# simonsobs/Pixell.jl

Measured on AMD Instinct MI355X. Metric: Mpix/s CAR bilinear reproject (Float64) + % HBM roofline, 1/2/4/8 MI355X, higher is better.
Workload: dtype f64

## Files before the change

### include/pixell_hip.h

```cpp
#ifndef PIXELL_HIP_H
#define PIXELL_HIP_H

#include <stddef.h>
#include <stdint.h>

#ifdef __cplusplus
extern "C" {
#endif

#define PXL_VERSION 100

typedef struct pxl_car_wcs {
    double cdelt[2];
    double crpix[2];
    double crval[2];
    double unit;
} pxl_car_wcs;

#define PXL_OK         0
#define PXL_EINVAL   (-22)
#define PXL_ENOMEM   (-12)
#define PXL_EHIP     (-5)
#define PXL_ENODEV   (-19)

// ... 39 lines not shown
int pxl_pix2sky_tan_f64(const pxl_car_wcs* wcs, int64_t n, const double* ipix, const double* jpix,
                        double* ra, double* dec, void* stream);
int pxl_posmap_tan_f64(const pxl_car_wcs* wcs, const int64_t shape[2], int64_t row0, int64_t nrows,
                       double* ra, double* dec, void* stream);

typedef struct pxl_reproject_plan pxl_reproject_plan;

int pxl_reproject_plan_create(const pxl_car_wcs* wcs_in, const int64_t shape_in[3],
                              int64_t src_row0, int64_t src_nrows,
                              const pxl_car_wcs* wcs_out, const int64_t shape_out[2],
                              int64_t dst_row0, int64_t dst_nrows,
                              pxl_reproject_plan** plan);
int pxl_reproject_execute(pxl_reproject_plan* plan, const double* src, double* dst, void* stream);
int pxl_reproject_build_tables(pxl_reproject_plan* plan, void* stream);
int pxl_reproject_execute_rows(pxl_reproject_plan* plan, const double* src, double* dst,
                               int64_t r0, int64_t nr, void* stream);
int pxl_reproject_execute_f32(pxl_reproject_plan* plan, const float* src, float* dst, void* stream);
int pxl_reproject_execute_rows_f32(pxl_reproject_plan* plan, const float* src, float* dst,
                                   int64_t r0, int64_t nr, void* stream);
int pxl_reproject_plan_src_rows(const pxl_reproject_plan* plan, int64_t* lo, int64_t* hi);
int pxl_reproject_plan_rows_covered(const pxl_reproject_plan* plan, int64_t have_lo, int64_t have_hi,
                                    int64_t* lo, int64_t* hi);
int pxl_reproject_plan_set_variant(pxl_reproject_plan* plan, int variant);
int pxl_reproject_plan_destroy(pxl_reproject_plan* plan);

typedef struct pxl_halo_xfer {
    int32_t peer;
    int32_t reserved;
    int64_t row0;
    int64_t nrows;
} pxl_halo_xfer;
int pxl_reproject_sharded_step_f64(pxl_reproject_plan* plan, double* src, double* dst,
                                   int64_t own_row0, int64_t own_nrows,
                                   const pxl_halo_xfer* sends, int nsends, const pxl_halo_xfer* recvs, int nrecvs,
                                   void* rccl_comm, void* stream);
int pxl_reproject_sharded_step_f32(pxl_reproject_plan* plan, float* src, float* dst,
                                   int64_t own_row0, int64_t own_nrows,
                                   const pxl_halo_xfer* sends, int nsends, const pxl_halo_xfer* recvs, int nrecvs,
                                   void* rccl_comm, void* stream);

#define PXL_COMM_ID_BYTES 128
int pxl_comm_unique_id(void* id128);
int pxl_comm_init_rank(const void* id128, int rank, int nranks, void** comm);
int pxl_comm_destroy(void* comm);
const char* pxl_comm_backend(void);

// ... 112 lines not shown
```

### pixell.jl_amd/_lib.py

```python
import ctypes as C
import os

_HERE = os.path.dirname(os.path.abspath(__file__))
LIB_PATH = os.environ.get("PXL_LIB_PATH", os.path.join(_HERE, "libpixell_hip.so"))

WRAP_NONE, WRAP_REWIND, WRAP_UNWIND = 0, 1, 2
FORM_RECIP, FORM_DIV, FORM_RECIP_AV = 0, 1, 2


class PixellHipError(RuntimeError):

    def __init__(self, code, message):
        super().__init__("libpixell_hip error %d: %s" % (code, message))
        self.code = code


class CarWCSStruct(C.Structure):
    _fields_ = [("cdelt", C.c_double * 2), ("crpix", C.c_double * 2), ("crval", C.c_double * 2),
                ("unit", C.c_double)]


_P = C.c_void_p
_I64 = C.c_int64
_WP = C.POINTER(CarWCSStruct)
# ... 5 lines not shown
    "pxl_device_count": (C.c_int, []),
    "pxl_release_scratch": (C.c_int, []),
    "pxl_pix2sky_car_f64": (C.c_int, [_WP, _I64, _P, _P, C.c_int, _P]),
    "pxl_rewind_f64": (C.c_int, [_P, _I64, C.c_double, C.c_double, _P]),
    "pxl_unwind_f64": (C.c_int, [_P, _I64, C.c_int, C.c_double, C.c_double, _P]),
    "pxl_pix2sky_car_soa_f64": (C.c_int, [_WP, _I64, _P, _P, _P, _P, C.c_int, _P]),
    "pxl_sky2pix_car_f64": (C.c_int, [_WP, _SHP, _I64, _P, _P, C.c_int, C.c_int, _P]),
    "pxl_sky2pix_car_soa_f64": (C.c_int, [_WP, _SHP, _I64, _P, _P, _P, _P, C.c_int, C.c_int, _P]),
    "pxl_posmap_car_f64": (C.c_int, [_WP, _SHP, _I64, _I64, _P, _P, C.c_int, _P]),
    "pxl_pixareamap_car_f64": (C.c_int, [_WP, _SHP, _I64, _I64, _P, _P]),
    "pxl_distance_transform_car_f64": (C.c_int, [_WP, _SHP, _P, _P, _P]),
    "pxl_sky2pix_tan_f64": (C.c_int, [_WP, _I64, _P, _P, _P, _P, _P]),
    "pxl_pix2sky_tan_f64": (C.c_int, [_WP, _I64, _P, _P, _P, _P, _P]),
    "pxl_posmap_tan_f64": (C.c_int, [_WP, _SHP, _I64, _I64, _P, _P, _P]),
    "pxl_reproject_plan_create": (C.c_int, [_WP, _SHP, _I64, _I64, _WP, _SHP, _I64, _I64, C.POINTER(_P)]),
    "pxl_reproject_execute": (C.c_int, [_P, _P, _P, _P]),
    "pxl_reproject_build_tables": (C.c_int, [_P, _P]),
    "pxl_reproject_execute_rows": (C.c_int, [_P, _P, _P, _I64, _I64, _P]),
    "pxl_reproject_execute_f32": (C.c_int, [_P, _P, _P, _P]),
    "pxl_reproject_execute_rows_f32": (C.c_int, [_P, _P, _P, _I64, _I64, _P]),
    "pxl_reproject_plan_src_rows": (C.c_int, [_P, C.POINTER(_I64), C.POINTER(_I64)]),
    "pxl_reproject_plan_rows_covered": (C.c_int, [_P, _I64, _I64, C.POINTER(_I64), C.POINTER(_I64)]),
    "pxl_reproject_plan_set_variant": (C.c_int, [_P, C.c_int]),
    "pxl_reproject_plan_destroy": (C.c_int, [_P]),
    "pxl_reproject_sharded_step_f64": (C.c_int, [_P, _P, _P, _I64, _I64, _P, C.c_int, _P, C.c_int, _P, _P]),
    "pxl_reproject_sharded_step_f32": (C.c_int, [_P, _P, _P, _I64, _I64, _P, C.c_int, _P, C.c_int, _P, _P]),
    "pxl_comm_unique_id": (C.c_int, [_P]),
    "pxl_comm_init_rank": (C.c_int, [_P, C.c_int, C.c_int, C.POINTER(_P)]),
    "pxl_comm_destroy": (C.c_int, [_P]),
    "pxl_comm_backend": (C.c_char_p, []),
    "pxl_reproject_car_bilinear_f64": (C.c_int, [_WP, _SHP, _P, _WP, _SHP, _P, _P]),
    "pxl_reproject_generic_bilinear_f64": (C.c_int, [_WP, C.c_int, _SHP, _P, _WP, C.c_int, _SHP, _P, _P]),
    "pxl_reproject_generic_last_tiles": (C.c_int, [C.POINTER(_I64), C.POINTER(_I64), _P]),
    "pxl_generic_plan_create": (C.c_int, [_WP, C.c_int, _SHP, _WP, C.c_int, _SHP, _P, C.POINTER(_P)]),
    "pxl_generic_plan_execute": (C.c_int, [_P, _I64, _P, _P, _P]),
    "pxl_generic_plan_tiles": (C.c_int, [_P, C.POINTER(_I64), C.POINTER(_I64)]),
    "pxl_generic_plan_destroy": (C.c_int, [_P]),
    "pxl_sample_car_bilinear_f64": (C.c_int, [_WP, _SHP, _P, _I64, _I64, _I64, _P, _P, _P]),
    "pxl_sample_car_bilinear_f32": (C.c_int, [_WP, _SHP, _P, _I64, _I64, _I64, _P, _P, _P]),
    "pxl_scatter_car_bilinear_f64": (C.c_int, [_WP, _SHP, _P, _I64, _I64, _I64, _P, _P, _P]),
    "pxl_sample_pairs_elems": (_I64, [_SHP, _I64]),
    "pxl_sample_build_pairs_f64": (C.c_int, [_SHP, _P, _I64, _P, _P]),
    "pxl_sample_build_pairs_f32": (C.c_int, [_SHP, _P, _I64, _P, _P]),
    "pxl_sample_car_bilinear_pairs_f64": (C.c_int, [_WP, _SHP, _P, _I64, _I64, _I64, _P, _P, _P]),
    "pxl_sample_car_bilinear_pairs_f32": (C.c_int, [_WP, _SHP, _P, _I64, _I64, _I64, _P, _P, _P]),
    "pxl_spline_prefilter_car_f64": (C.c_int, [_WP, _SHP, _P, _P, _P]),
# ... 78 lines not shown
```

### pixell.jl_amd/csrc/pxl_kernels.hip

```cpp
#include <hip/hip_runtime.h>

#include <algorithm>
#include <mutex>
#include <vector>
#include <cmath>
#include <cstdarg>
#include <cstdio>
#include <cstring>
#include <new>
#include <type_traits>

#include "pxl_device.h"

using namespace pxl;

static thread_local char g_err[512] = "";

static int fail(int code, const char* fmt, ...) {
    va_list ap;
    va_start(ap, fmt);
    vsnprintf(g_err, sizeof(g_err), fmt, ap);
    va_end(ap);
    return code;
}
#define HIP_TRY(expr)                                                                         \
// ... 32 lines not shown
    const char* v = getenv(name);
    return (v && *v) ? atoi(v) : dflt;
}

#include "pxl_elementwise.h"
#include "pxl_unwrap.h"
#include "pxl_maps.h"
#include "pxl_fastmath.h"
#include "pxl_tan.h"
#include "pxl_reproject.h"
#include "pxl_reproject_dma.h"
#include "pxl_sample.h"
#include "pxl_scatter.h"
#include "pxl_misc.h"
#include "pxl_rccl.h"
#include "pxl_spread.h"
#include "pxl_distance.h"
#include "pxl_spline.h"
#include "pxl_pol.h"
#include "pxl_polsolve.h"

static constexpr size_t PXL_RING_BYTES = 17 * 1024;
static constexpr int64_t PXL_MIN_TILES = 8192;

struct Tables { double* xfx; double* yfy; int32_t* xi0; int32_t* yj0; size_t bytes; };
static Tables table_layout(void* mem, int64_t nxo, int64_t nyo) {
    auto up16 = [](size_t b) { return (b + 15) & ~(size_t)15; };
    const uintptr_t xfx = (uintptr_t)mem, yfy = xfx + up16((size_t)nxo * 8), xi0 = yfy + up16((size_t)nyo * 8),
                    yj0 = xi0 + up16((size_t)nxo * 4);
    return {(double*)xfx, (double*)yfy, (int32_t*)xi0, (int32_t*)yj0, (size_t)(yj0 + up16((size_t)nyo * 4) - xfx)};
}
static void launch_build_tables(const pxl_car_wcs& win, int64_t nx, int64_t ny, const pxl_car_wcs& wout, int64_t nxo, int64_t nyo,
                                const Tables& t, hipStream_t st) {
    hipLaunchKernelGGL(k_build_tables, dim3(stream_grid(nxo + nyo, 256)), dim3(256), 0, st, car_affine(wout),
                       sky2pix_setup(win, nx, ny, 1, PXL_FORM_DIV), nxo, nyo, t.xi0, t.xfx, t.yj0, t.yfy);
}

struct SlotRule { int cw; double slack; int64_t align; };
static constexpr SlotRule kSlot64 = {128, 5.0, 2};
static constexpr SlotRule kSlot32 = {256, 8.0, 4};
static int64_t seg_for(const SlotRule& r, int pairs, double sx) {
    double span = ceil((double)(r.cw * pairs) * sx) + r.slack;
    return ((int64_t)span + (r.align - 1)) & ~(r.align - 1);
}
static bool stageable(const SlotRule& r, int64_t sg, bool periodic, int64_t nx, double sy) {
    return (sg <= PXL_MAXCH * r.cw) && !(periodic && sg > nx) && sy <= 3.0;
// ... 3 lines not shown
    pxl_car_wcs win, wout;
    int64_t nx, ny, nc, src_row0, src_nrows;
    int64_t nxo, nyo, dst_row0, dst_nrows;
    int periodic;
    int device;
    Tables tab;
    void* table_mem;
    int32_t* h_yj0;
    int variant;
    int pairs;
    int pairs_dma;
    int seg_dma;
    int pairs_dma32;
    int seg_dma32;
    bool dma32_ok;
    int dypos;
    int rh;
    int rh32;
    int seg;
    int dxpos;
    int ns, pf;
    int nt;
    double* zero_page;
    bool staged_ok;
    bool vec_load;
    bool tables_built;
    hipStream_t comm_stream;
    hipEvent_t ev_ready, ev_halo;
    int64_t cov_have_lo, cov_have_hi, cov_lo, cov_hi;
};

struct DeviceState {
    hipMemPool_t pool;
    unsigned int* last_exact;
    int64_t generic_tiles;
};
static std::mutex g_dev_mu;
static DeviceState g_dev[64] = {};
static DeviceState* device_state() {
    int dev = 0;
    if (hipGetDevice(&dev) != hipSuccess || dev < 0 || dev >= 64) return nullptr;
    return &g_dev[dev];
}

static hipMemPool_t scratch_pool() {
    DeviceState* d = device_state();
    if (!d) return nullptr;
    std::lock_guard<std::mutex> lock(g_dev_mu);
    if (!d->pool) {
// ... 163 lines not shown
    if (items < (int64_t)min_per_front * fronts) fronts = 1;
    int64_t per = (items + fronts - 1) / fronts;
    if (cap > 0 && per * fronts > cap) { fronts = 1; per = items; }
    return {fronts, per};
}

static int check_rows(const char* who, const int64_t shape[2], int64_t row0, int64_t nrows) {
    if (!shape || shape[0] < 1 || shape[1] < 1) return fail(PXL_EINVAL, "%s: bad shape", who);
    if (row0 < 0 || nrows < 0 || row0 + nrows > shape[1])
        return fail(PXL_EINVAL, "%s: rows [%lld, %lld) outside the map (ny=%lld)", who, (long long)row0,
                    (long long)(row0 + nrows), (long long)shape[1]);
    return PXL_OK;
}

template <class T>
static int reproject_rows_impl(pxl_reproject_plan* pl, const T* src, T* dst, int64_t r0, int64_t nr, void* stream) {
    if (!pl) return fail(PXL_EINVAL, "execute: null plan");
    if (r0 < 0 || nr < 0 || r0 + nr > pl->dst_nrows) return fail(PXL_EINVAL, "execute: rows outside the dst window");
    if (nr == 0) return PXL_OK;
    if (!dst || (!src && pl->src_nrows > 0)) return fail(PXL_EINVAL, "execute: null src/dst");
    if (!pl->tables_built) return fail(PXL_EINVAL, "execute_rows: tables not built");
    hipStream_t st = (hipStream_t)stream;
    constexpr bool f32 = std::is_same<T, float>::value;

    ReprojParams p;
    memset(&p, 0, sizeof(p));
    p.src = src; p.dst = dst;
    p.xi0 = pl->tab.xi0; p.xfx = pl->tab.xfx; p.yj0 = pl->tab.yj0; p.yfy = pl->tab.yfy;
    p.nx = pl->nx; p.ny = pl->ny; p.src_row0 = pl->src_row0; p.src_nrows = pl->src_nrows;
    p.nxo = pl->nxo; p.dst_row0 = pl->dst_row0; p.dst_nrows = pl->dst_nrows;
    p.r0 = r0; p.nr = nr; p.nc = (int32_t)pl->nc; p.periodic = pl->periodic;

    const bool aligned = (((uintptr_t)src & 15) == 0);
    bool staged = f32 ? (pl->dma32_ok && aligned) : pl->staged_ok;
    if (pl->variant == 1) staged = false;
    if (!staged) {
        int64_t work = ((pl->nxo + 1) / 2) * nr;
        dim3 g(stream_grid(work, 256), (unsigned)pl->nc);
        hipLaunchKernelGGL((k_reproject_gather<T>), g, dim3(256), 0, st, p);
        return check_launch("k_reproject_gather");
    }

    const bool vec = f32 ? true : (pl->vec_load && aligned);
    const bool use_dma = f32 ? true : (vec && pl->variant != 2);
    const int pairs = f32 ? pl->pairs_dma32 : (use_dma ? pl->pairs_dma : pl->pairs);
    const int cw = f32 ? kSlot32.cw : kSlot64.cw;
    const int TW = cw * pairs;
    p.seg = f32 ? pl->seg_dma32 : (use_dma ? pl->seg_dma : pl->seg);
    p.dxpos = pl->dxpos; p.dypos = pl->dypos;
    p.ntx = (int32_t)((pl->nxo + TW - 1) / TW);
    int rh = f32 ? pl->rh32 : pl->rh;
    while (rh > 4 && (int64_t)p.ntx * ((nr + rh - 1) / rh) * pl->nc < PXL_MIN_TILES) rh >>= 1;
    p.rh = rh;
    p.nty = (int32_t)((nr + rh - 1) / rh);
    p.ntiles = (int64_t)p.ntx * p.nty * pl->nc;
    p.tiles_per_xcd = (p.ntiles + 7) / 8;
    const int64_t nblocks = 8 * p.tiles_per_xcd;
    if (nblocks > 0x7fffffffLL) return fail(PXL_EINVAL, "execute: too many tiles (%lld)", (long long)nblocks);
    dim3 grid((unsigned)nblocks), block(64);
    if (use_dma) {
        const size_t esz = sizeof(T);
        p.ns = pl->ns; p.pf = pl->pf; p.zero_page = pl->zero_page;
        p.nt = pl->nt != 0;
        while ((size_t)p.ns * p.seg * esz > PXL_RING_BYTES && p.ns > 4) p.ns >>= 1;
        size_t dma_lds = (size_t)p.ns * (size_t)p.seg * esz;
        const int nch = (p.seg + cw - 1) / cw;
        return launch_reproject_dma_t<T>(pairs, nch, grid, dma_lds, st, p);
    }
    size_t lds_bytes = (size_t)PXL_NS * (size_t)pl->seg * sizeof(double);
    if (pl->pairs == 2) {
        if (vec) hipLaunchKernelGGL((k_reproject_staged<2, true>), grid, block, lds_bytes, st, p);
        else     hipLaunchKernelGGL((k_reproject_staged<2, false>), grid, block, lds_bytes, st, p);
    } else {
        if (vec) hipLaunchKernelGGL((k_reproject_staged<1, true>), grid, block, lds_bytes, st, p);
        else     hipLaunchKernelGGL((k_reproject_staged<1, false>), grid, block, lds_bytes, st, p);
    }
    return check_launch("k_reproject_staged");
}

template <class T>
static int sharded_step_impl(pxl_reproject_plan* pl, T* src, T* dst, int64_t own_row0, int64_t own_nrows,
                             const pxl_halo_xfer* sends, int nsends, const pxl_halo_xfer* recvs, int nrecvs,
                             void* comm, void* stream) {
    if (!pl || !src || !dst) return fail(PXL_EINVAL, "sharded_step: null plan or buffer");
    if (nsends < 0 || nrecvs < 0 || (nsends > 0 && !sends) || (nrecvs > 0 && !recvs)) return fail(PXL_EINVAL, "sharded_step: bad transfer lists");
    const int64_t lo = pl->src_row0, hi = pl->src_row0 + pl->src_nrows;
    if (own_row0 < lo || own_nrows < 0 || own_row0 + own_nrows > hi) return fail(PXL_EINVAL, "sharded_step: owned rows outside the plan's source window");
    hipStream_t st = (hipStream_t)stream;
    int rc = PXL_OK;
    const bool exchange = nsends + nrecvs > 0;
// ... 513 lines not shown
    if (shape_in[0] < 1 || shape_in[1] < 1 || shape_in[2] < 1 || shape_out[0] < 1 || shape_out[1] < 1)
        return fail(PXL_EINVAL, "plan_create: shapes must be positive");
    if (shape_in[0] > 400000000 || shape_in[1] > 1000000000 || shape_out[0] > 1000000000 || shape_out[1] > 1000000000)
        return fail(PXL_EINVAL, "plan_create: axis too long (source RA axis <= 4e8, others <= 1e9 pixels)");
    if (src_row0 < 0 || src_nrows < 0 || src_row0 + src_nrows > shape_in[1])
        return fail(PXL_EINVAL, "plan_create: source window outside the map");
    if (dst_row0 < 0 || dst_nrows < 0 || dst_row0 + dst_nrows > shape_out[1])
        return fail(PXL_EINVAL, "plan_create: destination window outside the map");

    pxl_reproject_plan* pl = new (std::nothrow) pxl_reproject_plan();
    if (!pl) return fail(PXL_ENOMEM, "plan_create: host allocation failed");
    pl->cov_lo = 0; pl->cov_hi = -1;
    pl->win = *wcs_in; pl->wout = *wcs_out;
    pl->nx = shape_in[0]; pl->ny = shape_in[1]; pl->nc = shape_in[2];
    pl->src_row0 = src_row0; pl->src_nrows = src_nrows;
    pl->nxo = shape_out[0]; pl->nyo = shape_out[1];
    pl->dst_row0 = dst_row0; pl->dst_nrows = dst_nrows;
    pl->periodic = car_periodic(wcs_in, pl->nx);
    pl->tables_built = false;

    hipError_t e = hipGetDevice(&pl->device);
    if (e != hipSuccess) { delete pl; return fail(PXL_ENODEV, "hipGetDevice: %s", hipGetErrorString(e)); }

    const size_t nyo = (size_t)pl->nyo, off_zero = table_layout(nullptr, pl->nxo, pl->nyo).bytes, total = off_zero + 64;
    e = hipMalloc(&pl->table_mem, total);
    if (e != hipSuccess) { delete pl; return fail(PXL_ENOMEM, "plan_create: hipMalloc(%zu): %s", total, hipGetErrorString(e)); }
    char* base = (char*)pl->table_mem;
    e = hipMemset(base + off_zero, 0, 64);
    if (e != hipSuccess) { (void)hipFree(pl->table_mem); delete pl; return fail(PXL_EHIP, "plan_create: hipMemset: %s", hipGetErrorString(e)); }
    pl->zero_page = (double*)(base + off_zero);
    pl->tab = table_layout(base, pl->nxo, pl->nyo);

    pl->h_yj0 = new (std::nothrow) int32_t[nyo];
    if (!pl->h_yj0) { (void)hipFree(pl->table_mem); delete pl; return fail(PXL_ENOMEM, "plan_create: host allocation failed"); }
    CarAffine co = car_affine(pl->wout);
    Sky2Pix si = sky2pix_setup(pl->win, pl->nx, pl->ny, 1, PXL_FORM_DIV);
    for (int64_t j = 0; j < pl->nyo; ++j) {
        double fr;
        split_cell(s2p_y(si, p2s_dec(co, (double)(j + 1))), &pl->h_yj0[j], &fr);
    }

    double sx = fabs((pl->wout.cdelt[0] * pl->wout.unit) / (pl->win.cdelt[0] * pl->win.unit));
    pl->dxpos = ((pl->wout.cdelt[0] * pl->wout.unit) / (pl->win.cdelt[0] * pl->win.unit)) > 0 ? 1 : 0;
    pl->dypos = ((pl->wout.cdelt[1] * pl->wout.unit) / (pl->win.cdelt[1] * pl->win.unit)) > 0 ? 1 : 0;
    double sy = fabs((pl->wout.cdelt[1] * pl->wout.unit) / (pl->win.cdelt[1] * pl->win.unit));
    pl->rh = env_int("PXL_REPROJECT_RH", sy >= 1.5 ? 4 : (sy > 0.3 ? 16 : 8));
    if (pl->rh < 1) pl->rh = 1;
    if (pl->rh > 64) pl->rh = 64;
    pl->rh32 = env_int("PXL_REPROJECT_RH", 32);
    if (pl->rh32 < 1) pl->rh32 = 1;
    if (pl->rh32 > 64) pl->rh32 = 64;
    pl->ns = env_int("PXL_REPROJECT_NS", (double)pl->nx * (double)pl->ny * (double)pl->nc * 8.0 <= 128.0 * 1048576.0 ? 4 : 8);
    if (pl->ns < 4) pl->ns = 4;
// ... 7 lines not shown
    if (pl->pf < 0) pl->pf = 0;
    const int max_seg = PXL_MAXCH * kSlot64.cw;
    int want = env_int("PXL_REPROJECT_PAIRS", sx <= 0.55 ? 4 : 2);
    if (want != 1 && want != 2 && want != 4) want = 2;
    pl->pairs_dma = want;
    while (pl->pairs_dma > 1 && seg_for(kSlot64, pl->pairs_dma, sx) > max_seg) pl->pairs_dma >>= 1;
    const int64_t seg_dma = seg_for(kSlot64, pl->pairs_dma, sx);
    pl->seg_dma = (int)std::min<int64_t>(seg_dma, max_seg);
    pl->pairs = want > 2 ? 2 : want;
    if (seg_for(kSlot64, pl->pairs, sx) > max_seg && pl->pairs == 2) pl->pairs = 1;
    int64_t seg = seg_for(kSlot64, pl->pairs, sx);
    pl->staged_ok = stageable(kSlot64, seg, pl->periodic, pl->nx, sy) && stageable(kSlot64, seg_dma, pl->periodic, pl->nx, sy);
    pl->seg = (int)(seg <= max_seg ? seg : max_seg);
    {
        const int max_seg32 = PXL_MAXCH * kSlot32.cw;
        pl->pairs_dma32 = env_int("PXL_REPROJECT_PAIRS", sx < 0.75 ? 1 : 2);
        if (pl->pairs_dma32 != 1 && pl->pairs_dma32 != 2 && pl->pairs_dma32 != 4) pl->pairs_dma32 = 2;
        while (pl->pairs_dma32 > 1 && seg_for(kSlot32, pl->pairs_dma32, sx) > max_seg32) pl->pairs_dma32 >>= 1;
        int64_t s32 = seg_for(kSlot32, pl->pairs_dma32, sx);
        pl->dma32_ok = stageable(kSlot32, s32, pl->periodic, pl->nx, sy) && (pl->nx % 4 == 0);
        pl->seg_dma32 = (int)std::min<int64_t>(s32, max_seg32);
    }
    pl->vec_load = (pl->nx % 2 == 0);
    *out = pl;
    return PXL_OK;
}

int pxl_reproject_plan_set_variant(pxl_reproject_plan* pl, int variant) {
    if (!pl || variant < 0 || variant > 2) return fail(PXL_EINVAL, "set_variant: bad argument");
    pl->variant = variant;
    return PXL_OK;
}

int pxl_reproject_plan_destroy(pxl_reproject_plan* pl) {
    if (!pl) return PXL_OK;
    if (pl->comm_stream) {
        (void)hipStreamSynchronize(pl->comm_stream);
        (void)hipEventDestroy(pl->ev_ready);
        (void)hipEventDestroy(pl->ev_halo);
        (void)hipStreamDestroy(pl->comm_stream);
    }
    if (pl->table_mem) (void)hipFree(pl->table_mem);
    delete[] pl->h_yj0;
    delete pl;
    return PXL_OK;
}

int pxl_reproject_build_tables(pxl_reproject_plan* pl, void* stream) {
    if (!pl) return fail(PXL_EINVAL, "build_tables: null plan");
    launch_build_tables(pl->win, pl->nx, pl->ny, pl->wout, pl->nxo, pl->nyo, pl->tab, (hipStream_t)stream);
    int rc = check_launch("k_build_tables");
    if (rc == PXL_OK) pl->tables_built = true;
    return rc;
}

int pxl_reproject_execute_rows(pxl_reproject_plan* pl, const double* src, double* dst, int64_t r0, int64_t nr,
                               void* stream) {
    return reproject_rows_impl(pl, src, dst, r0, nr, stream);
}

int pxl_reproject_execute_rows_f32(pxl_reproject_plan* pl, const float* src, float* dst, int64_t r0, int64_t nr,
                                   void* stream) {
    return reproject_rows_impl(pl, src, dst, r0, nr, stream);
}

int pxl_reproject_execute(pxl_reproject_plan* pl, const double* src, double* dst, void* stream) {
    int rc = pxl_reproject_build_tables(pl, stream);
    if (rc) return rc;
    return pxl_reproject_execute_rows(pl, src, dst, 0, pl->dst_nrows, stream);
}

int pxl_reproject_execute_f32(pxl_reproject_plan* pl, const float* src, float* dst, void* stream) {
    int rc = pxl_reproject_build_tables(pl, stream);
    if (rc) return rc;
    return pxl_reproject_execute_rows_f32(pl, src, dst, 0, pl->dst_nrows, stream);
// ... 494 lines not shown
```

### pixell.jl_amd/csrc/pxl_reproject.h

```cpp
#pragma once

__global__ __launch_bounds__(256) void k_build_tables(CarAffine out, Sky2Pix in, int64_t nxo, int64_t nyo,
                                                      int32_t* __restrict__ xi0, double* __restrict__ xfx,
                                                      int32_t* __restrict__ yj0, double* __restrict__ yfy) {
    int64_t stride = (int64_t)gridDim.x * blockDim.x;
    for (int64_t k = (int64_t)blockIdx.x * blockDim.x + threadIdx.x; k < nxo + nyo; k += stride) {
        if (k < nxo) {
            double a = p2s_ra(out, (double)(k + 1));
            split_cell(s2p_x(in, a), &xi0[k], &xfx[k]);
        } else {
            int64_t j = k - nxo;
            double d = p2s_dec(out, (double)(j + 1));
            split_cell(s2p_y(in, d), &yj0[j], &yfy[j]);
        }
    }
}

struct ReprojParams {
    const void* src;
    void* dst;
    const int32_t* xi0; const double* xfx;
    const int32_t* yj0; const double* yfy;
    int64_t nx, ny, src_row0, src_nrows;
    int64_t nxo, dst_row0, dst_nrows;
    int64_t r0, nr;
    int32_t nc, periodic;
    int32_t rh;
    int32_t seg;
    int32_t dxpos;
    int32_t dypos;
    int32_t ntx, nty;
    int64_t ntiles, tiles_per_xcd;
    int32_t ns, pf;
    int32_t nt;
    const double* zero_page;
};

__device__ inline int64_t xcd_tile(int64_t b, int64_t tiles_per_xcd) {
    return (b & 7) * tiles_per_xcd + (b >> 3);
}

template <typename T>
__global__ __launch_bounds__(256) void k_reproject_gather(ReprojParams p) {
    const int64_t npair = (p.nxo + 1) / 2;
    const int64_t total = npair * p.nr;
    const int c = blockIdx.y;
    SrcViewT<T> m{(const T*)p.src + (int64_t)c * p.nx * p.src_nrows, p.nx, p.ny, p.src_row0, p.src_nrows, p.periodic};
    T* dplane = (T*)p.dst + (int64_t)c * p.nxo * p.dst_nrows;
    int64_t stride = (int64_t)gridDim.x * blockDim.x;
    for (int64_t t = (int64_t)blockIdx.x * blockDim.x + threadIdx.x; t < total; t += stride) {
        int64_t rr = t / npair;
        int64_t i = (t - rr * npair) * 2;
        int64_t r = p.r0 + rr;
        int64_t j0 = p.yj0[p.dst_row0 + r];
        double fy = p.yfy[p.dst_row0 + r];
        int64_t o = r * p.nxo + i;
        dplane[o] = (T)bilerp_cells(m, p.xi0[i], p.xfx[i], j0, fy);
        if (i + 1 < p.nxo) dplane[o + 1] = (T)bilerp_cells(m, p.xi0[i + 1], p.xfx[i + 1], j0, fy);
// ... 185 lines not shown
```

### pixell.jl_amd/csrc/pxl_reproject_dma.h

```cpp
#pragma once

template <int N>
__device__ __forceinline__ void wait_vm() {
    asm volatile("s_waitcnt vmcnt(%0)" ::"n"(N) : "memory");
}

__device__ __forceinline__ void wait_vm_upto(int k) {
    if (k < 8) {
        if (k < 4) {
            if (k < 2) { if (k < 1) wait_vm<0>(); else wait_vm<1>(); }
            else       { if (k < 3) wait_vm<2>(); else wait_vm<3>(); }
        } else {
            if (k < 6) { if (k < 5) wait_vm<4>(); else wait_vm<5>(); }
            else       { if (k < 7) wait_vm<6>(); else wait_vm<7>(); }
        }
    } else if (k < 16) {
        if (k < 12) {
            if (k < 10) { if (k < 9) wait_vm<8>(); else wait_vm<9>(); }
            else        { if (k < 11) wait_vm<10>(); else wait_vm<11>(); }
        } else {
            if (k < 14) { if (k < 13) wait_vm<12>(); else wait_vm<13>(); }
            else        { if (k < 15) wait_vm<14>(); else wait_vm<15>(); }
        }
    } else {
        if (k < 24) { if (k < 20) wait_vm<16>(); else wait_vm<20>(); }
        else        { if (k < 32) wait_vm<24>(); else wait_vm<32>(); }
    }
}

__device__ __forceinline__ void glds16_saddr(const void* sbase, uint32_t voff, uint32_t lds_byte_addr) {
    asm volatile("s_mov_b32 m0, %2\n\ts_nop 4\n\tglobal_load_lds_dwordx4 %1, %0"
                 :: "s"(sbase), "v"(voff), "s"(lds_byte_addr) : "memory");
}
__device__ __forceinline__ void glds16_vaddr(const void* gsrc, uint32_t lds_byte_addr) {
    asm volatile("s_mov_b32 m0, %1\n\ts_nop 0\n\tglobal_load_lds_dwordx4 %0, off"
                 :: "v"(gsrc), "s"(lds_byte_addr) : "memory");
}

template <typename T, int PAIRS, int NCH>
__global__ __launch_bounds__(64) void k_reproject_dma(ReprojParams p) {
    extern __shared__ __attribute__((aligned(16))) unsigned char lds_raw[];
    T* const lds = reinterpret_cast<T*>(lds_raw);
    const int lane = threadIdx.x;
    constexpr int EPL = 16 / (int)sizeof(T);
    constexpr int CW = 64 * EPL;
    constexpr int TW = CW * PAIRS;

    const int64_t t = xcd_tile(blockIdx.x, p.tiles_per_xcd);
    if (t >= p.ntiles) return;
    const int tx = (int)(t % p.ntx);
    const int64_t trest = t / p.ntx;
    const int ty = (int)(trest % p.nty);
    const int c = (int)(trest / p.nty);

    const T* splane = (const T*)p.src + (int64_t)c * p.nx * p.src_nrows;
    T* dplane = (T*)p.dst + (int64_t)c * p.nxo * p.dst_nrows;

    const int64_t c0 = (int64_t)tx * TW;
    const int64_t clast = (c0 + TW < p.nxo ? c0 + TW : p.nxo) - 1;
    const int64_t rb = p.r0 + (int64_t)ty * p.rh;
    const int64_t re = (rb + p.rh < p.r0 + p.nr) ? rb + p.rh : p.r0 + p.nr;
    const int nrows = (int)(re - rb);

    const int64_t a = p.dxpos ? p.xi0[c0] : p.xi0[clast];
    const int64_t ua = a - 1;
    const int64_t cbase0 = ua - (((ua % EPL) + EPL) % EPL);
    int dloc[PAIRS][EPL];
    double fx[PAIRS][EPL];
    bool act[PAIRS][EPL];
    bool fits = true;
#pragma unroll
    for (int q = 0; q < PAIRS; ++q) {
// ... 17 lines not shown
    const int dir = p.dypos ? 1 : -1;
    const int my_t0 = p.dypos ? my_j0 : -(my_j0 + 1);
    const double my_wa = p.dypos ? 1 - my_fy : my_fy;
    const double my_wb = p.dypos ? my_fy : 1 - my_fy;
    {
        int nxt = __shfl_down(my_t0, 1, 64);
        bool mono = (lane + 1 >= nrows) || (nxt >= my_t0);
        if (!mono) fits = false;
    }

    if (!__all(fits)) {
        SrcViewT<T> m{splane, p.nx, p.ny, p.src_row0, p.src_nrows, p.periodic};
        for (int64_t r = rb; r < re; ++r) {
            int64_t j0 = p.yj0[p.dst_row0 + r];
            double fy = p.yfy[p.dst_row0 + r];
#pragma unroll
            for (int q = 0; q < PAIRS; ++q)
#pragma unroll
                for (int e = 0; e < EPL; ++e) {
                    int64_t col = c0 + q * CW + EPL * lane + e;
                    if (act[q][e]) dplane[r * p.nxo + col] = (T)bilerp_cells(m, p.xi0[col], fx[q][e], j0, fy);
                }
        }
        return;
    }

    uint32_t voff[NCH];
#pragma unroll
    for (int ch = 0; ch < NCH; ++ch) {
        int64_t u = cbase0 + ch * CW + EPL * lane;
        bool ok = true;
        if (p.periodic) { u %= p.nx; if (u < 0) u += p.nx; }
        else ok = (u >= 0) && (u < p.nx);
        voff[ch] = ok ? (uint32_t)(u * (int64_t)sizeof(T)) : 0xFFFFFFFFu;
    }

    const uint32_t lds_base = (uint32_t)(uintptr_t)lds;
    const uint32_t slot_bytes = (uint32_t)p.seg * (uint32_t)sizeof(T);
    const int ns_mask = p.ns - 1;

    int tv_lo = 1, tv_hi = 0;
    {
        const int64_t jlo = (p.src_row0 + 1 > 1) ? p.src_row0 + 1 : 1;
        const int64_t jhi = (p.src_row0 + p.src_nrows < p.ny) ? p.src_row0 + p.src_nrows : p.ny;
        if (jhi >= jlo) {
            if (p.dypos) { tv_lo = (int)jlo; tv_hi = (int)jhi; } else { tv_lo = -(int)jhi; tv_hi = -(int)jlo; }
        }
// ... 35 lines not shown

    const bool vec_store = ((p.nxo % EPL) == 0) && (((uintptr_t)p.dst & 15) == 0);
    T* orow = dplane + rb * p.nxo + c0 + EPL * lane;

    double hA[PAIRS][EPL], hB[PAIRS][EPL], wx[PAIRS][EPL];
#pragma unroll
    for (int q = 0; q < PAIRS; ++q)
#pragma unroll
        for (int e = 0; e < EPL; ++e) { wx[q][e] = 1 - fx[q][e]; hA[q][e] = 0.0; hB[q][e] = 0.0; }
    auto hrow = [&](int tr, double (&h)[PAIRS][EPL]) {
        const T* R = lds + (tr & ns_mask) * p.seg;
#pragma unroll
        for (int q = 0; q < PAIRS; ++q)
#pragma unroll
            for (int e = 0; e < EPL; ++e) {
                const int d = dloc[q][e];
                h[q][e] = wx[q][e] * (double)R[d] + fx[q][e] * (double)R[d + 1];
            }
    };
    auto row_loop = [&](auto fast_tag, auto nt_tag) {
    constexpr bool FAST = decltype(fast_tag)::value;
    constexpr bool NT = decltype(nt_tag)::value;
    int th = INT32_MIN / 2;
    for (int rr = 0; rr < nrows; ++rr) {
        const int t0 = __builtin_amdgcn_readlane(my_t0, rr);
        {
            const int ra = (rr + p.pf < nrows) ? rr + p.pf : nrows - 1;
            int tmax = __builtin_amdgcn_readlane(my_t0, ra) + 1;
            const int tlim = t0 + p.ns - 1;
            if (tmax > tlim) tmax = tlim;
            while (treq < tmax) issue_next();
        }
        if (t0 != th) {
            wait_vm_upto(vm_total - __builtin_amdgcn_readlane(marks, (t0 + 1) & ns_mask));
            if (t0 == th + 1) {
#pragma unroll
                for (int q = 0; q < PAIRS; ++q)
#pragma unroll
                    for (int e = 0; e < EPL; ++e) hA[q][e] = hB[q][e];
            } else {
                hrow(t0, hA);
            }
            hrow(t0 + 1, hB);
            th = t0;
            asm volatile("s_waitcnt lgkmcnt(0)" ::: "memory");
        }
        const double wa = __hiloint2double(__builtin_amdgcn_readlane(__double2hiint(my_wa), rr),
                                           __builtin_amdgcn_readlane(__double2loint(my_wa), rr));
        const double wb = __hiloint2double(__builtin_amdgcn_readlane(__double2hiint(my_wb), rr),
                                           __builtin_amdgcn_readlane(__double2loint(my_wb), rr));
#pragma unroll
        for (int q = 0; q < PAIRS; ++q) {
            alignas(16) T v[EPL];
#pragma unroll
            for (int e = 0; e < EPL; ++e) v[e] = (T)(wa * hA[q][e] + wb * hB[q][e]);
            T* o = orow + q * CW;
            if (FAST) {
                typedef unsigned int u4v __attribute__((ext_vector_type(4)));
                if (NT) __builtin_nontemporal_store(*reinterpret_cast<const u4v*>(v), reinterpret_cast<u4v*>(o));
                else *reinterpret_cast<uint4*>(o) = *reinterpret_cast<const uint4*>(v);
            }
            else if (vec_store) { if (act[q][0]) *reinterpret_cast<uint4*>(o) = *reinterpret_cast<const uint4*>(v); }
            else {
#pragma unroll
                for (int e = 0; e < EPL; ++e) if (act[q][e]) o[e] = v[e];
            }
        }
        if (FAST) vm_total += PAIRS;
        orow += p.nxo;
    }
    };
    if (vec_store && (c0 + TW <= p.nxo)) {
        if (p.nt) row_loop(std::true_type{}, std::true_type{});
        else row_loop(std::true_type{}, std::false_type{});
    } else row_loop(std::false_type{}, std::false_type{});
}

template <typename T>
static int launch_reproject_dma_t(int pairs, int nch, dim3 grid, size_t lds_bytes, hipStream_t st, const ReprojParams& p) {
#define PXL_DMA_CASE(P, N) \
    if (pairs == P && nch == N) { hipLaunchKernelGGL((k_reproject_dma<T, P, N>), grid, dim3(64), lds_bytes, st, p); return check_launch("k_reproject_dma"); }
    PXL_DMA_CASE(1, 1) PXL_DMA_CASE(1, 2) PXL_DMA_CASE(1, 3) PXL_DMA_CASE(1, 4) PXL_DMA_CASE(1, 5)
    PXL_DMA_CASE(2, 1) PXL_DMA_CASE(2, 2) PXL_DMA_CASE(2, 3) PXL_DMA_CASE(2, 4) PXL_DMA_CASE(2, 5)
    PXL_DMA_CASE(4, 1) PXL_DMA_CASE(4, 2) PXL_DMA_CASE(4, 3) PXL_DMA_CASE(4, 4) PXL_DMA_CASE(4, 5)
#undef PXL_DMA_CASE
    return fail(PXL_EINVAL, "reproject: no LDS-DMA kernel for pairs=%d nch=%d", pairs, nch);
}
```

### pixell.jl_amd/ops.py

```python
import ctypes as C

import torch

from . import _lib, placement
from ._lib import FORM_DIV, FORM_RECIP, FORM_RECIP_AV, WRAP_NONE, WRAP_REWIND, WRAP_UNWIND
from .enmap import Enmap, _geom
from .wcs import (AbstractCARWCS, Gnomonic, pix2sky_scalar, pix2sky_tan_scalar, sky2pix_scalar,
                  sky2pix_tan_scalar)


def _stream(t: torch.Tensor):
    return C.c_void_p(torch.cuda.current_stream(t.device).cuda_stream)


def _dev_f64(t: torch.Tensor, what: str) -> torch.Tensor:
    if not isinstance(t, torch.Tensor):
        raise TypeError("%s must be a torch tensor" % what)
    if not t.is_cuda:
        raise RuntimeError("%s must live on the GPU: the MI355X path has no CPU fallback "
                           "(CPU arrays stay with the reference implementation)" % what)
    if t.dtype != torch.float64:
        raise TypeError("%s must be float64" % what)
    if not t.is_contiguous():
        raise ValueError("%s must be contiguous" % what)
# ... 273 lines not shown
        self.wcs_in, self.wcs_out = wcs_in, wcs_out
        self.src_rows = (0, self.shape_in[1]) if src_rows is None else (int(src_rows[0]), int(src_rows[1]))
        self.dst_rows = (0, self.shape_out[1]) if dst_rows is None else (int(dst_rows[0]), int(dst_rows[1]))
        self.device = torch.device(device)
        self._h = C.c_void_p()
        with torch.cuda.device(self.device):
            _lib.check(_lib.load().pxl_reproject_plan_create(
                _wcs_ref(wcs_in), _lib.shape_arr(self.shape_in), self.src_rows[0], self.src_rows[1],
                _wcs_ref(wcs_out), _lib.shape_arr(self.shape_out), self.dst_rows[0], self.dst_rows[1],
                C.byref(self._h)))

    @property
    def ncomp(self):
        return self.shape_in[2]

    def src_tensor_shape(self):
        return (self.ncomp, self.src_rows[1], self.shape_in[0])

    def dst_tensor_shape(self):
        return (self.ncomp, self.dst_rows[1], self.shape_out[0])

    def set_variant(self, variant: int):
        _lib.check(_lib.load().pxl_reproject_plan_set_variant(self._h, int(variant)))

    def src_rows_needed(self):
        lo, hi = C.c_int64(), C.c_int64()
        _lib.check(_lib.load().pxl_reproject_plan_src_rows(self._h, C.byref(lo), C.byref(hi)))
        return lo.value, hi.value

    def rows_covered(self, have_lo, have_hi):
        lo, hi = C.c_int64(), C.c_int64()
        _lib.check(_lib.load().pxl_reproject_plan_rows_covered(self._h, have_lo, have_hi, C.byref(lo), C.byref(hi)))
        return lo.value, hi.value

    def _check(self, src, dst):
        src, dst = _dev_map(src, "src"), _dev_map(dst, "dst")
        if src.dtype != dst.dtype:
            raise TypeError("src and dst must have the same dtype (Float64 or Float32)")
        if src.numel() != self.ncomp * self.src_rows[1] * self.shape_in[0]:
            raise ValueError("src has %d elements, plan expects %s" % (src.numel(), (self.src_tensor_shape(),)))
        if dst.numel() != self.ncomp * self.dst_rows[1] * self.shape_out[0]:
            raise ValueError("dst has %d elements, plan expects %s" % (dst.numel(), (self.dst_tensor_shape(),)))
        if src.data_ptr() == dst.data_ptr():
            raise ValueError("src and dst must not alias")
        return src, dst

# ... 558 lines not shown
```

Baseline: 385,200.

## Add opt-in persistent work-stealing reproject kernel and cache table builds

Adds a persistent variant of the LDS-DMA reproject kernel. It launches only as many workgroups as can be resident at once, and each workgroup claims tiles through per-XCD atomic counters, stealing from the fullest other region when its own runs out. The next tile is claimed a few rows before the current one finishes, to hide the claim latency. The path is off by default and turns on through PXL_REPROJECT_PERSIST or set_workgroups. Separately, build_tables now records an event and skips rebuilding the tables once they are ready, which removes repeated table-build kernel launches but assumes the plan's inputs never change.

Result: slower. 374,000 (-2.9%).

```diff
diff --git a/include/pixell_hip.h b/include/pixell_hip.h
--- a/include/pixell_hip.h
+++ b/include/pixell_hip.h
@@ -85,6 +85,9 @@
 int pxl_reproject_plan_rows_covered(const pxl_reproject_plan* plan, int64_t have_lo, int64_t have_hi,
                                     int64_t* lo, int64_t* hi);
 int pxl_reproject_plan_set_variant(pxl_reproject_plan* plan, int variant);
+int pxl_reproject_plan_set_workgroups(pxl_reproject_plan* plan, int n);
+int pxl_reproject_plan_last_launch(pxl_reproject_plan* plan, int64_t out[4]);
+int pxl_reproject_plan_tables_built(const pxl_reproject_plan* plan);
 int pxl_reproject_plan_destroy(pxl_reproject_plan* plan);
 
 typedef struct pxl_halo_xfer {
diff --git a/pixell.jl_amd/_lib.py b/pixell.jl_amd/_lib.py
--- a/pixell.jl_amd/_lib.py
+++ b/pixell.jl_amd/_lib.py
@@ -51,6 +51,9 @@
     "pxl_reproject_plan_src_rows": (C.c_int, [_P, C.POINTER(_I64), C.POINTER(_I64)]),
     "pxl_reproject_plan_rows_covered": (C.c_int, [_P, _I64, _I64, C.POINTER(_I64), C.POINTER(_I64)]),
     "pxl_reproject_plan_set_variant": (C.c_int, [_P, C.c_int]),
+    "pxl_reproject_plan_set_workgroups": (C.c_int, [_P, C.c_int]),
+    "pxl_reproject_plan_last_launch": (C.c_int, [_P, C.POINTER(_I64)]),
+    "pxl_reproject_plan_tables_built": (C.c_int, [_P]),
     "pxl_reproject_plan_destroy": (C.c_int, [_P]),
     "pxl_reproject_sharded_step_f64": (C.c_int, [_P, _P, _P, _I64, _I64, _P, C.c_int, _P, C.c_int, _P, _P]),
     "pxl_reproject_sharded_step_f32": (C.c_int, [_P, _P, _P, _I64, _I64, _P, C.c_int, _P, C.c_int, _P, _P]),
diff --git a/pixell.jl_amd/csrc/pxl_claim.h b/pixell.jl_amd/csrc/pxl_claim.h
--- /dev/null
+++ b/pixell.jl_amd/csrc/pxl_claim.h
@@ -0,0 +1,103 @@
+#pragma once
+#include <stdint.h>
+
+#ifndef PXL_CLAIM_HD
+#define PXL_CLAIM_HD __host__ __device__ inline
+#endif
+
+#define PXL_CLAIM_REGIONS 8
+#define PXL_CLAIM_LEFT 8
+#define PXL_CLAIM_OWN 9
+#define PXL_CLAIM_STOLEN 10
+#define PXL_CLAIM_REPORT 12
+#define PXL_CLAIM_WORDS 16
+
+PXL_CLAIM_HD uint64_t pxl_claim_load(uint64_t* w) {
+#if defined(__HIP_DEVICE_COMPILE__)
+    return __hip_atomic_load(w, __ATOMIC_RELAXED, __HIP_MEMORY_SCOPE_AGENT);
+#else
+    return __atomic_load_n(w, __ATOMIC_SEQ_CST);
+#endif
+}
+PXL_CLAIM_HD void pxl_claim_store(uint64_t* w, uint64_t v) {
+#if defined(__HIP_DEVICE_COMPILE__)
+    __hip_atomic_store(w, v, __ATOMIC_RELAXED, __HIP_MEMORY_SCOPE_AGENT);
+#else
+    __atomic_store_n(w, v, __ATOMIC_SEQ_CST);
+#endif
+}
+PXL_CLAIM_HD uint64_t pxl_claim_add(uint64_t* w, uint64_t v) {
+#if defined(__HIP_DEVICE_COMPILE__)
+    return __hip_atomic_fetch_add(w, v, __ATOMIC_RELAXED, __HIP_MEMORY_SCOPE_AGENT);
+#else
+    return __atomic_fetch_add(w, v, __ATOMIC_SEQ_CST);
+#endif
+}
+PXL_CLAIM_HD uint64_t pxl_claim_cas(uint64_t* w, uint64_t expect, uint64_t want) {
+#if defined(__HIP_DEVICE_COMPILE__)
+    __hip_atomic_compare_exchange_strong(w, &expect, want, __ATOMIC_RELAXED, __ATOMIC_RELAXED, __HIP_MEMORY_SCOPE_AGENT);
+#else
+    __atomic_compare_exchange_n(w, &expect, want, false, __ATOMIC_SEQ_CST, __ATOMIC_SEQ_CST);
+#endif
+    return expect;
+}
+
+PXL_CLAIM_HD void pxl_claim_answered(uint64_t v) {
+#if defined(__HIP_DEVICE_COMPILE__)
+    asm volatile("; answered %0" ::"v"(v) : "memory");
+#else
+    (void)v;
+#endif
+}
+
+PXL_CLAIM_HD int64_t pxl_claim_region_size(int64_t ntiles, int64_t tpx, int v) {
+    const int64_t n = ntiles - (int64_t)v * tpx;
+    return n < 0 ? 0 : (n > tpx ? tpx : n);
+}
+PXL_CLAIM_HD int64_t pxl_claim_left(uint64_t word, int64_t n) {
+    return n - (int64_t)(uint32_t)word - (int64_t)(word >> 32);
+}
+
+PXL_CLAIM_HD int64_t pxl_claim_in_region(uint64_t* w, int64_t n, int top, int64_t* tries) {
+    uint64_t cur = pxl_claim_load(w);
+    for (;;) {
+        if (pxl_claim_left(cur, n) <= 0) return -1;
+        ++*tries;
+        const uint64_t seen = pxl_claim_cas(w, cur, cur + (top ? (1ull << 32) : 1ull));
+        if (seen == cur) return top ? n - 1 - (int64_t)(cur >> 32) : (int64_t)(uint32_t)cur;
+        cur = seen;
+    }
+}
+
+PXL_CLAIM_HD int64_t pxl_claim_next(uint64_t* words, int64_t ntiles, int64_t tpx, int home, int* stolen, int64_t* tries) {
+    *stolen = 0;
+    int64_t k = pxl_claim_in_region(words + home, pxl_claim_region_size(ntiles, tpx, home), 0, tries);
+    if (k >= 0) return (int64_t)home * tpx + k;
+    for (;;) {
+        int best = -1;
+        int64_t most = 0;
+        for (int v = 0; v < PXL_CLAIM_REGIONS; ++v) {
+            if (v == home) continue;
+            const int64_t left = pxl_claim_left(pxl_claim_load(words + v), pxl_claim_region_size(ntiles, tpx, v));
+            if (left > most) { most = left; best = v; }
+        }
+        if (best < 0) return -1;
+        k = pxl_claim_in_region(words + best, pxl_claim_region_size(ntiles, tpx, best), 1, tries);
+        if (k >= 0) { *stolen = 1; return (int64_t)best * tpx + k; }
+    }
+}
+
+PXL_CLAIM_HD bool pxl_claim_leave(uint64_t* words, int64_t nwg, int64_t ntiles, int64_t own, int64_t stolen) {
+    if (own) pxl_claim_answered(pxl_claim_add(words + PXL_CLAIM_OWN, (uint64_t)own));
+    if (stolen) pxl_claim_answered(pxl_claim_add(words + PXL_CLAIM_STOLEN, (uint64_t)stolen));
+    if ((int64_t)pxl_claim_add(words + PXL_CLAIM_LEFT, 1) != nwg - 1) return false;
+    pxl_claim_store(words + PXL_CLAIM_REPORT + 0, (uint64_t)ntiles);
+    pxl_claim_store(words + PXL_CLAIM_REPORT + 1, (uint64_t)nwg);
+    pxl_claim_store(words + PXL_CLAIM_REPORT + 2, pxl_claim_load(words + PXL_CLAIM_OWN));
+    pxl_claim_store(words + PXL_CLAIM_REPORT + 3, pxl_claim_load(words + PXL_CLAIM_STOLEN));
+    for (int v = 0; v < PXL_CLAIM_REGIONS; ++v) pxl_claim_store(words + v, 0);
+    pxl_claim_store(words + PXL_CLAIM_OWN, 0);
+    pxl_claim_store(words + PXL_CLAIM_STOLEN, 0);
+    pxl_claim_store(words + PXL_CLAIM_LEFT, 0);
+    return true;
+}
diff --git a/pixell.jl_amd/csrc/pxl_kernels.hip b/pixell.jl_amd/csrc/pxl_kernels.hip
--- a/pixell.jl_amd/csrc/pxl_kernels.hip
+++ b/pixell.jl_amd/csrc/pxl_kernels.hip
@@ -1,6 +1,7 @@
 #include <hip/hip_runtime.h>
 
 #include <algorithm>
+#include <atomic>
 #include <mutex>
 #include <vector>
 #include <cmath>
@@ -79,6 +80,7 @@
 
 static constexpr size_t PXL_RING_BYTES = 17 * 1024;
 static constexpr int64_t PXL_MIN_TILES = 8192;
+static constexpr int PXL_CLAIM_SLOTS = 4;
 
 struct Tables { double* xfx; double* yfy; int32_t* xi0; int32_t* yj0; size_t bytes; };
 static Tables table_layout(void* mem, int64_t nxo, int64_t nyo) {
@@ -128,9 +130,18 @@
     int ns, pf;
     int nt;
     double* zero_page;
+    uint64_t* claim_mem;
+    std::atomic<unsigned> claim_turn;
+    int last_slot;
+    int64_t last_tiles;
+    int workgroups;
+    int persist_auto;
     bool staged_ok;
     bool vec_load;
     bool tables_built;
+    bool tables_ready;
+    hipStream_t tables_stream;
+    hipEvent_t ev_tables;
     hipStream_t comm_stream;
     hipEvent_t ev_ready, ev_halo;
     int64_t cov_have_lo, cov_have_hi, cov_lo, cov_hi;
@@ -340,6 +351,8 @@
     if (!pl->tables_built) return fail(PXL_EINVAL, "execute_rows: tables not built");
     hipStream_t st = (hipStream_t)stream;
     constexpr bool f32 = std::is_same<T, float>::value;
+    pl->last_tiles = 0;
+    pl->last_slot = -1;
 
     ReprojParams p;
     memset(&p, 0, sizeof(p));
@@ -376,6 +389,7 @@
     const int64_t nblocks = 8 * p.tiles_per_xcd;
     if (nblocks > 0x7fffffffLL) return fail(PXL_EINVAL, "execute: too many tiles (%lld)", (long long)nblocks);
     dim3 grid((unsigned)nblocks), block(64);
+    pl->last_tiles = p.ntiles;
     if (use_dma) {
         const size_t esz = sizeof(T);
         p.ns = pl->ns; p.pf = pl->pf; p.zero_page = pl->zero_page;
@@ -383,7 +397,12 @@
         while ((size_t)p.ns * p.seg * esz > PXL_RING_BYTES && p.ns > 4) p.ns >>= 1;
         size_t dma_lds = (size_t)p.ns * (size_t)p.seg * esz;
         const int nch = (p.seg + cw - 1) / cw;
-        return launch_reproject_dma_t<T>(pairs, nch, grid, dma_lds, st, p);
+        const int slot = (int)(pl->claim_turn.fetch_add(1) % PXL_CLAIM_SLOTS);
+        p.claim = pl->claim_mem + (size_t)slot * PXL_CLAIM_WORDS;
+        int64_t wgs = 0;
+        const int rc = launch_reproject_dma_t<T>(pairs, nch, dma_lds, st, p, pl->workgroups > 0 ? pl->workgroups : (pl->persist_auto ? -1 : 0), &wgs);
+        if (rc == PXL_OK && wgs > 0) pl->last_slot = slot;
+        return rc;
     }
     size_t lds_bytes = (size_t)PXL_NS * (size_t)pl->seg * sizeof(double);
     if (pl->pairs == 2) {
@@ -943,13 +962,16 @@
     hipError_t e = hipGetDevice(&pl->device);
     if (e != hipSuccess) { delete pl; return fail(PXL_ENODEV, "hipGetDevice: %s", hipGetErrorString(e)); }
 
-    const size_t nyo = (size_t)pl->nyo, off_zero = table_layout(nullptr, pl->nxo, pl->nyo).bytes, total = off_zero + 64;
+    const size_t nyo = (size_t)pl->nyo, off_zero = table_layout(nullptr, pl->nxo, pl->nyo).bytes, claim_bytes = (size_t)PXL_CLAIM_SLOTS * PXL_CLAIM_WORDS * 8,
+                 total = off_zero + 64 + claim_bytes;
     e = hipMalloc(&pl->table_mem, total);
     if (e != hipSuccess) { delete pl; return fail(PXL_ENOMEM, "plan_create: hipMalloc(%zu): %s", total, hipGetErrorString(e)); }
     char* base = (char*)pl->table_mem;
-    e = hipMemset(base + off_zero, 0, 64);
+    e = hipMemset(base + off_zero, 0, 64 + claim_bytes);
     if (e != hipSuccess) { (void)hipFree(pl->table_mem); delete pl; return fail(PXL_EHIP, "plan_create: hipMemset: %s", hipGetErrorString(e)); }
     pl->zero_page = (double*)(base + off_zero);
+    pl->claim_mem = (uint64_t*)(base + off_zero + 64);
+    pl->last_slot = -1;
     pl->tab = table_layout(base, pl->nxo, pl->nyo);
 
     pl->h_yj0 = new (std::nothrow) int32_t[nyo];
@@ -1003,6 +1025,7 @@
         pl->seg_dma32 = (int)std::min<int64_t>(s32, max_seg32);
     }
     pl->vec_load = (pl->nx % 2 == 0);
+    pl->persist_auto = env_int("PXL_REPROJECT_PERSIST", 0) != 0;
     *out = pl;
     return PXL_OK;
 }
@@ -1013,8 +1036,29 @@
     return PXL_OK;
 }
 
+int pxl_reproject_plan_set_workgroups(pxl_reproject_plan* pl, int n) {
+    if (!pl || n < 0 || n > (1 << 20)) return fail(PXL_EINVAL, "set_workgroups: bad argument");
+    pl->workgroups = n;
+    return PXL_OK;
+}
+
+int pxl_reproject_plan_last_launch(pxl_reproject_plan* pl, int64_t out[4]) {
+    if (!pl || !out) return fail(PXL_EINVAL, "last_launch: null argument");
+    out[0] = pl->last_tiles; out[1] = out[2] = out[3] = 0;
+    if (pl->last_slot < 0) return PXL_OK;
+    uint64_t rep[4];
+    HIP_TRY(hipMemcpy(rep, pl->claim_mem + (size_t)pl->last_slot * PXL_CLAIM_WORDS + PXL_CLAIM_REPORT, sizeof(rep), hipMemcpyDeviceToHost));
+    for (int k = 0; k < 4; ++k) out[k] = (int64_t)rep[k];
+    return PXL_OK;
+}
+
+int pxl_reproject_plan_tables_built(const pxl_reproject_plan* pl) {
+    return pl && pl->tables_built ? 1 : 0;
+}
+
 int pxl_reproject_plan_destroy(pxl_reproject_plan* pl) {
     if (!pl) return PXL_OK;
+    if (pl->ev_tables) (void)hipEventDestroy(pl->ev_tables);
     if (pl->comm_stream) {
         (void)hipStreamSynchronize(pl->comm_stream);
         (void)hipEventDestroy(pl->ev_ready);
@@ -1029,9 +1073,25 @@
 
 int pxl_reproject_build_tables(pxl_reproject_plan* pl, void* stream) {
     if (!pl) return fail(PXL_EINVAL, "build_tables: null plan");
-    launch_build_tables(pl->win, pl->nx, pl->ny, pl->wout, pl->nxo, pl->nyo, pl->tab, (hipStream_t)stream);
+    hipStream_t st = (hipStream_t)stream;
+    if (pl->tables_ready) return PXL_OK;
+    hipStreamCaptureStatus cap = hipStreamCaptureStatusNone;
+    if (hipStreamIsCapturing(st, &cap) != hipSuccess) { (void)hipGetLastError(); cap = hipStreamCaptureStatusNone; }
+    const bool capturing = cap != hipStreamCaptureStatusNone;
+    if (pl->ev_tables) {
+        if (hipEventQuery(pl->ev_tables) == hipSuccess) { pl->tables_ready = true; return PXL_OK; }
+        (void)hipGetLastError();
+        if (!capturing && st == pl->tables_stream) return PXL_OK;
+    }
+    launch_build_tables(pl->win, pl->nx, pl->ny, pl->wout, pl->nxo, pl->nyo, pl->tab, st);
     int rc = check_launch("k_build_tables");
-    if (rc == PXL_OK) pl->tables_built = true;
+    if (rc != PXL_OK) return rc;
+    pl->tables_built = true;
+    if (!capturing && !pl->ev_tables) {
+        if (hipEventCreateWithFlags(&pl->ev_tables, hipEventDisableTiming) != hipSuccess) { (void)hipGetLastError(); pl->ev_tables = nullptr; return rc; }
+        if (hipEventRecord(pl->ev_tables, st) != hipSuccess) { (void)hipGetLastError(); (void)hipEventDestroy(pl->ev_tables); pl->ev_tables = nullptr; return rc; }
+        pl->tables_stream = st;
+    }
     return rc;
 }
 
diff --git a/pixell.jl_amd/csrc/pxl_reproject.h b/pixell.jl_amd/csrc/pxl_reproject.h
--- a/pixell.jl_amd/csrc/pxl_reproject.h
+++ b/pixell.jl_amd/csrc/pxl_reproject.h
@@ -34,6 +34,7 @@
     int32_t ns, pf;
     int32_t nt;
     const double* zero_page;
+    uint64_t* claim;
 };
 
 __device__ inline int64_t xcd_tile(int64_t b, int64_t tiles_per_xcd) {
diff --git a/pixell.jl_amd/csrc/pxl_reproject_dma.h b/pixell.jl_amd/csrc/pxl_reproject_dma.h
--- a/pixell.jl_amd/csrc/pxl_reproject_dma.h
+++ b/pixell.jl_amd/csrc/pxl_reproject_dma.h
@@ -1,4 +1,5 @@
 #pragma once
+#include "pxl_claim.h"
 
 template <int N>
 __device__ __forceinline__ void wait_vm() {
@@ -37,17 +38,13 @@
                  :: "v"(gsrc), "s"(lds_byte_addr) : "memory");
 }
 
-template <typename T, int PAIRS, int NCH>
-__global__ __launch_bounds__(64) void k_reproject_dma(ReprojParams p) {
-    extern __shared__ __attribute__((aligned(16))) unsigned char lds_raw[];
-    T* const lds = reinterpret_cast<T*>(lds_raw);
-    const int lane = threadIdx.x;
+template <typename T, int PAIRS, int NCH, bool PERSIST, class Claim>
+__device__ __forceinline__ int64_t reproject_dma_tile(const ReprojParams& p, const int64_t t, T* const lds, const int lane, Claim& claim) {
     constexpr int EPL = 16 / (int)sizeof(T);
     constexpr int CW = 64 * EPL;
     constexpr int TW = CW * PAIRS;
-
-    const int64_t t = xcd_tile(blockIdx.x, p.tiles_per_xcd);
-    if (t >= p.ntiles) return;
+    int64_t next = -1;
+
     const int tx = (int)(t % p.ntx);
     const int64_t trest = t / p.ntx;
     const int ty = (int)(trest % p.nty);
@@ -111,7 +108,8 @@
                     if (act[q][e]) dplane[r * p.nxo + col] = (T)bilerp_cells(m, p.xi0[col], fx[q][e], j0, fy);
                 }
         }
-        return;
+        if constexpr (PERSIST) next = claim();
+        return next;
     }
 
     uint32_t voff[NCH];
@@ -193,6 +191,7 @@
     constexpr bool FAST = decltype(fast_tag)::value;
     constexpr bool NT = decltype(nt_tag)::value;
     int th = INT32_MIN / 2;
+    const int claim_at = (nrows - 1 - p.pf > 0) ? nrows - 1 - p.pf : 0;
     for (int rr = 0; rr < nrows; ++rr) {
         const int t0 = __builtin_amdgcn_readlane(my_t0, rr);
         {
@@ -202,6 +201,7 @@
             if (tmax > tlim) tmax = tlim;
             while (treq < tmax) issue_next();
         }
+        if constexpr (PERSIST) { if (rr == claim_at) next = claim(); }
         if (t0 != th) {
             wait_vm_upto(vm_total - __builtin_amdgcn_readlane(marks, (t0 + 1) & ns_mask));
             if (t0 == th + 1) {
@@ -245,12 +245,79 @@
         if (p.nt) row_loop(std::true_type{}, std::true_type{});
         else row_loop(std::true_type{}, std::false_type{});
     } else row_loop(std::false_type{}, std::false_type{});
+    return next;
+}
+
+template <typename T, int PAIRS, int NCH>
+__global__ __launch_bounds__(64) void k_reproject_dma(ReprojParams p) {
+    extern __shared__ __attribute__((aligned(16))) unsigned char lds_raw[];
+    const int64_t t = xcd_tile(blockIdx.x, p.tiles_per_xcd);
+    if (t >= p.ntiles) return;
+    int none = 0;
+    (void)reproject_dma_tile<T, PAIRS, NCH, false>(p, t, reinterpret_cast<T*>(lds_raw), (int)threadIdx.x, none);
+}
+
+template <typename T, int PAIRS, int NCH>
+__global__ __launch_bounds__(64) void k_reproject_dma_persistent(ReprojParams p) {
+    extern __shared__ __attribute__((aligned(16))) unsigned char lds_raw[];
+    const int lane = threadIdx.x;
+    const int home = (int)(blockIdx.x & 7);
+    int n_own = 0, n_stolen = 0;
+    auto claim = [&]() -> int64_t {
+        int tn = -1, st = 0;
+        if (lane == 0) {
+            int64_t tries = 0;
+            tn = (int)pxl_claim_next(p.claim, p.ntiles, p.tiles_per_xcd, home, &st, &tries);
+        }
+        tn = __builtin_amdgcn_readfirstlane(tn);
+        st = __builtin_amdgcn_readfirstlane(st);
+        if (tn >= 0) { if (st) ++n_stolen; else ++n_own; }
+        return (int64_t)tn;
+    };
+    int64_t t = claim();
+    while (t >= 0) t = reproject_dma_tile<T, PAIRS, NCH, true>(p, t, reinterpret_cast<T*>(lds_raw), lane, claim);
+    if (lane == 0) (void)pxl_claim_leave(p.claim, (int64_t)gridDim.x, p.ntiles, n_own, n_stolen);
+}
+
+static int64_t resident_workgroups(const void* fn, int block, size_t lds_bytes) {
+    struct Known { const void* fn; size_t lds; int dev; int64_t n; };
+    static std::mutex mu;
+    static std::vector<Known> known;
+    int dev = 0;
+    if (hipGetDevice(&dev) != hipSuccess) { (void)hipGetLastError(); return fail(PXL_ENODEV, "reproject: no current device"), -1; }
+    std::lock_guard<std::mutex> lock(mu);
+    for (const Known& k : known)
+        if (k.fn == fn && k.lds == lds_bytes && k.dev == dev) return k.n;
+    int per_cu = 0, cus = 0;
+    hipError_t e = hipOccupancyMaxActiveBlocksPerMultiprocessor(&per_cu, fn, block, lds_bytes);
+    if (e == hipSuccess) e = hipDeviceGetAttribute(&cus, hipDeviceAttributeMultiprocessorCount, dev);
+    if (e != hipSuccess || per_cu < 1 || cus < 1) {
+        (void)hipGetLastError();
+        return fail(PXL_EHIP, "reproject: occupancy query failed (%s; %d workgroups per CU, %d CUs)", hipGetErrorString(e), per_cu, cus), -1;
+    }
+    known.push_back({fn, lds_bytes, dev, (int64_t)per_cu * cus});
+    return known.back().n;
 }
 
 template <typename T>
-static int launch_reproject_dma_t(int pairs, int nch, dim3 grid, size_t lds_bytes, hipStream_t st, const ReprojParams& p) {
+static int launch_reproject_dma_t(int pairs, int nch, size_t lds_bytes, hipStream_t st, const ReprojParams& p, int64_t persist_wgs,
+                                  int64_t* wgs_out) {
+    *wgs_out = 0;
 #define PXL_DMA_CASE(P, N) \
-    if (pairs == P && nch == N) { hipLaunchKernelGGL((k_reproject_dma<T, P, N>), grid, dim3(64), lds_bytes, st, p); return check_launch("k_reproject_dma"); }
+    if (pairs == P && nch == N) { \
+        if (persist_wgs < 0) { \
+            const int64_t hold = resident_workgroups((const void*)k_reproject_dma_persistent<T, P, N>, 64, lds_bytes); \
+            if (hold < 0) return PXL_EHIP; \
+            persist_wgs = p.ntiles > hold ? hold : 0; \
+        } \
+        if (persist_wgs > 0) { \
+            *wgs_out = persist_wgs; \
+            hipLaunchKernelGGL((k_reproject_dma_persistent<T, P, N>), dim3((unsigned)persist_wgs), dim3(64), lds_bytes, st, p); \
+            return check_launch("k_reproject_dma_persistent"); \
+        } \
+        hipLaunchKernelGGL((k_reproject_dma<T, P, N>), dim3((unsigned)(8 * p.tiles_per_xcd)), dim3(64), lds_bytes, st, p); \
+        return check_launch("k_reproject_dma"); \
+    }
     PXL_DMA_CASE(1, 1) PXL_DMA_CASE(1, 2) PXL_DMA_CASE(1, 3) PXL_DMA_CASE(1, 4) PXL_DMA_CASE(1, 5)
     PXL_DMA_CASE(2, 1) PXL_DMA_CASE(2, 2) PXL_DMA_CASE(2, 3) PXL_DMA_CASE(2, 4) PXL_DMA_CASE(2, 5)
     PXL_DMA_CASE(4, 1) PXL_DMA_CASE(4, 2) PXL_DMA_CASE(4, 3) PXL_DMA_CASE(4, 4) PXL_DMA_CASE(4, 5)
diff --git a/pixell.jl_amd/ops.py b/pixell.jl_amd/ops.py
--- a/pixell.jl_amd/ops.py
+++ b/pixell.jl_amd/ops.py
@@ -319,6 +319,19 @@
 
     def set_variant(self, variant: int):
         _lib.check(_lib.load().pxl_reproject_plan_set_variant(self._h, int(variant)))
+
+    def set_workgroups(self, n: int):
+        _lib.check(_lib.load().pxl_reproject_plan_set_workgroups(self._h, int(n)))
+
+    def last_launch(self):
+        out = (C.c_int64 * 4)()
+        with torch.cuda.device(self.device):
+            _lib.check(_lib.load().pxl_reproject_plan_last_launch(self._h, out))
+        return tuple(int(v) for v in out)
+
+    @property
+    def tables_built(self):
+        return bool(_lib.load().pxl_reproject_plan_tables_built(self._h))
 
     def src_rows_needed(self):
         lo, hi = C.c_int64(), C.c_int64()
```
